# denyingmxd/CFPNet

Hardware: AMD Instinct MI355X
Metric: depth maps/sec @ 480x640 bf16 (whole job; per_gpu = value / n_gpus); abs_rel vs CPU oracle (higher is better)
Workload: dtype bf16; 1 GPU; batch=8 480x640 RGB + 8x8-zone ToF, eval forward incl. the prob output [B,256,H/2,W/2] written in the storage dtype (bf16: 2 bytes/element); layers=hist2image combine1 image x2 (CFPNet), parallelism=single GPU

## Files before the change

cfpnet_amd/csrc/conv_route.hip:

```cpp
#include "conv_route.h"

namespace {

int tile_count(int variant, int M, int Cout) {
  static const int bm[4] = {256, 256, 128, 128}, bn[4] = {16, 32, 64, 128};
  return cdiv(M, bm[variant]) * cdiv(Cout, bn[variant]);
}

int pick_splits(int variant, int M, int Cout, int K, int dtype) {
  const int bk = is16(dtype) ? 32 : 16;
  const int nk = cdiv(K, bk);
  const int tiles = tile_count(variant, M, Cout);
  if (tiles >= 128 || nk < 16) return 1;
  int s = cdiv(256, tiles);
  if (s > nk / 6) s = nk / 6;
  if (s > 32) s = 32;
  return s < 2 ? 1 : s;
}

}

static int g_force_variant = -1, g_force_splits = -1;
int g_use_v1 = 0;
int g_tput = 0;
// ... 14 lines not shown
static int chunk_x3_variant(long long M, int Cin, int Cout, bool tput) {
  if (Cin % 32 != 0) return -1;
  if (Cin == 32) {
    if (Cout <= 32) return M >= 30000 ? 45 : -1;
    if (Cout > 64 && Cout <= 128 && !tput) return (M >= 30000 && M < 200000) ? 44 : -1;
    return -1;
  }
  if (Cout > 128) return (tput && M >= 9000) ? 36 : -1;
  if (Cout > 64) return M >= 30000 ? ((!tput && M < 200000) ? 44 : 36) : -1;
  if (Cout <= 32) return M >= (tput ? 30000 : 15000) ? 45 : -1;
  if (M >= 100000) return 38;
  if (M >= 30000) return tput ? 38 : 24;
  return -1;
}
int g_chunk16 = 1;
static int chunk16_variant(long long M, int Cin, int Cout, bool tput) {
  if (Cin <= 64 || Cin % 8 != 0 || Cout <= 0 || Cout % 8 != 0 || M <= 0 || g_chunk16 == 0) return -1;
  if (g_chunk16 == 2) return Cout > 64 ? 0 : 1;
  if (M >= 30000 && M < 200000) return 1;
  if (M >= 8000 && M < 12000) return (Cout > 128) != tput ? 1 : -1;
  return -1;
}
extern "C" int cfp_conv3x3_chunk_variant(int M, int Cin, int Cout, int in_flight) { return chunk16_variant(M, Cin, Cout, in_flight > 1); }
static bool halo_wins_s2(long long M, int Cout) { return g_halo == 2 || (g_halo == 1 && g_halo_s2 && M >= 30000 && Cout <= 160); }
static bool halo_wins(long long M, int Cout, bool tput) {
  if (g_halo == 2) return true;
  if (g_halo == 1 && tput && M >= 100000 && Cout <= 64) return true;
  return g_halo == 1 && ((M >= 300000 && (Cout <= 32 || Cout == 128)) || (M >= 100000 && Cout > 128 && Cout <= 160) ||
                         (M >= 30000 && Cout > 160 && Cout <= 256));
}
void cfp_tail_x3_debug_set(int value);
void cfp_fold_debug_set(int v);
void cfp_tail16_debug_set(int value);
void cfp_pw_rows_debug_set(int value);
void cfp_attn_apply_debug_set(int value);
void cfp_dwl3_debug_set(int value);
void cfp_dwl_wgrad_debug_set(int value);
void cfp_wgrad_debug_set(int value);
void cfp_bn_debug_set(int key, int value);
void cfp_attn_debug_set(int value);
int cfp_dw_debug_set(int key, int value);
extern "C" int cfp_debug_set(int key, int value) {
  switch (key) {
    case 3: case 4: case 5: case 6: case 9: case 10: case 11: return cfp_dw_debug_set(key, value);
    case 30: cfp_dwl3_debug_set(value); return CFP_OK;
    case 32: g_x3_occ = value; return CFP_OK;
    case 33: g_x3_small_m = value; return CFP_OK;
    case 34: g_x3_small_k = value; return CFP_OK;
    case 35: cfp_tail_x3_debug_set(value); return CFP_OK;
    case 37: cfp_fold_debug_set(value); return CFP_OK;
    case 38: cfp_attn_apply_debug_set(value); return CFP_OK;
    case 39: cfp_tail16_debug_set(value); return CFP_OK;
    case 40: g_chunk16 = value; return CFP_OK;
    case 41: cfp_pw_rows_debug_set(value); return CFP_OK;
    case 17: g_tput = value; return CFP_OK;
    case 16: g_probe = (g_probe & 16) | value; return CFP_OK;
    case 29: g_x3_ad = value; return CFP_OK;
    case 28: g_probe = (g_probe & ~16) | (value ? 16 : 0); return CFP_OK;
    case 15: g_small_s2 = value; return CFP_OK;
    case 14: g_up_halo = value; return CFP_OK;
    case 19: cfp_attn_debug_set(value); return CFP_OK;
    case 20: case 21: cfp_bn_debug_set(key, value); return CFP_OK;
    case 22: cfp_wgrad_debug_set(value); return CFP_OK;
    case 23: cfp_dwl_wgrad_debug_set(value); return CFP_OK;
    case 18: g_halo_s2 = value; return CFP_OK;
    case 12: g_halo = value; return CFP_OK;
    case 24: g_halo_x3 = value; return CFP_OK;
    case 25: g_bin_head_x3_rows = value; return CFP_OK;
    case 26: g_x3_ln_fused = value; return CFP_OK;
    case 27: conv3x3_halo_debug_odd_pitch(value); return CFP_OK;
    case 13: conv3x3_halo_debug_stages(value); return CFP_OK;
    case 0: g_force_variant = value; return CFP_OK;
    case 1: g_force_splits = value; return CFP_OK;
    case 2: g_use_v1 = value; return CFP_OK;
    default: cfp_set_error("cfp_debug_set: unknown key"); return CFP_EINVAL;
  }
}

extern "C" int cfp_conv2d_variant(int M, int Cout) {
  if (Cout <= 16) return 0;
  if (Cout <= 32) return 1;
  if (Cout <= 64) return 2;
  long long t128 = (long long)cdiv(M, 128) * cdiv(Cout, 128);
  bool waste = (Cout % 128) != 0 && (Cout % 128) <= 64;
  return (t128 < 192 || waste) ? 2 : 3;
}

// ... 231 lines not shown
```

cfpnet_amd/csrc/loftr_tail.hip:

```cpp
#include "tail_core.h"

namespace {

template <typename H, int NT, int BSTAGE, int WAVES, typename AF>
__device__ __forceinline__ void tail_gemm(f32x4 (&acc)[NT], const H* __restrict__ W, int K, AF afrag, unsigned char* sB,
                                          int wave, int lane) {
  constexpr int N = NT * 16;
  constexpr int NBG = N / 8;
  constexpr int NBW = (NBG + WAVES - 1) / WAVES;
  constexpr int SST = N * 128;
  constexpr int STG = (3 * SST <= 2 * BSTAGE) ? 3 : 2;
  const int fr = lane & 15, fq = lane >> 4;
  const int rsub = lane >> 3;
  const int lc = (lane & 7) ^ rsub;
  const H* zsrc = reinterpret_cast<const H*>(g_zero16);
#pragma unroll
  for (int j = 0; j < NT; ++j) acc[j] = f32x4{0.f, 0.f, 0.f, 0.f};
  const int nk = (K + 63) >> 6;
  auto issue = [&](int ks, int st) {
    const int kk = ks * 64 + lc * 8;
    const bool kok = kk < K;
#pragma unroll
    for (int j = 0; j < NBW; ++j) {
      const int g = (j * WAVES + wave) % NBG;
// ... 129 lines not shown
    }
  }
  asm volatile("s_waitcnt lgkmcnt(0)" ::: "memory");

  constexpr int PF = D + 4;
  float* tF = reinterpret_cast<float*>(tH);
  {
    f32x4 acc[D / 16];
    tail_gemm<H, D / 16, BSTAGE, 4>(acc, p.w2, 4 * D, [&](int k) { return *reinterpret_cast<const s16x8*>(tH + fr * PH + k + fq * 8); }, sB, wave, lane);
    asm volatile("s_waitcnt lgkmcnt(0)" ::: "memory");
#pragma unroll
    for (int j = 0; j < D / 16; ++j) {
      const float bj = p.b2[j * 16 + fr];
#pragma unroll
      for (int r = 0; r < 4; ++r) tF[(fq * 4 + r) * PF + j * 16 + fr] = acc[j][r] + bj;
    }
  }
  asm volatile("s_waitcnt lgkmcnt(0)" ::: "memory");
  for (int i = lane; i < 16 * XCH; i += 64) {
    const int r = i / XCH, ch = i - r * XCH;
    const long long m = row0 + r;
    if (m < p.rows) {
      float a[8], b[8];
      Vec<float>::load(tF + r * PF + ch * 8, a);
      Vec<float>::load(tF + r * PF + ch * 8 + 4, a + 4);
      Vec<H>::load(p.xin + m * p.x_ld + ch * 8, b);
#pragma unroll
      for (int e = 0; e < 8; ++e) a[e] += b[e];
      Vec<H>::store(p.out + m * p.out_ld + ch * 8, a);
    }
  }
}

int g_tail16_waves = 0;

}

void cfp_tail16_debug_set(int value) { g_tail16_waves = value; }

static int loftr_tail_impl(const void* q, int q_ld, const float* kv, const float* ksum, const void* x, int x_ld,
                           void* out, int out_ld, const void* w_q, const void* w_merge, const void* w_mlp0, const void* w_mlp2,
                           const float* ln1_g, const float* ln1_b, const float* ln2_g, const float* ln2_b, float ln_eps,
                           int NB, int Hq, int Wq, int qth, int qtw, float v_length, float eps, int heads, int D,
                           int dtype, cfp_stream_t stream, const TailMap* map) {
  const bool x3 = dtype == CFP_F32X3;
  const int vec = x3 ? 4 : 8;
  const bool rows_ok = (long long)NB * Hq * Wq < (1ll << 31);
  CFP_REQUIRE(x3 || is16(dtype), CFP_EINVAL, "cfp_loftr_tail: bf16 / f16 or CFP_F32X3 (the plain f32 parity mode uses the unfused kernels)");
  CFP_REQUIRE((q || w_q) && kv && ksum && x && out && w_merge && w_mlp0 && w_mlp2 && ln1_g && ln1_b && ln2_g && ln2_b, CFP_EINVAL,
              "cfp_loftr_tail: null pointer (q or w_q must be given)");
  CFP_REQUIRE(NB > 0 && Hq > 0 && Wq > 0 && qth > 0 && qtw > 0 && v_length > 0.f && (rows_ok || !x3), CFP_ESHAPE, "cfp_loftr_tail: bad grid");
  CFP_REQUIRE((D == 32 || D == 64 || D == 128) && (heads == 4 || heads == 8), CFP_ESHAPE, "cfp_loftr_tail: D must be 32/64/128 and heads 4/8");
  CFP_REQUIRE((w_q || (q_ld >= D && q_ld % vec == 0)) && x_ld >= D && out_ld >= D && x_ld % vec == 0 && out_ld % vec == 0, CFP_ESHAPE,
              "cfp_loftr_tail: pitches must be >= D and multiples of " + std::to_string(vec));
  CFP_REQUIRE(aligned16(q) && aligned16(w_q) && aligned16(x) && aligned16(out) && aligned16(w_merge) && aligned16(w_mlp0) && aligned16(w_mlp2) &&
                  aligned16(kv), CFP_EINVAL, "cfp_loftr_tail: pointers must be 16-byte aligned");
  CFP_REQUIRE(rows_ok, CFP_ESHAPE, "cfp_loftr_tail: too many rows");
  hipStream_t s = reinterpret_cast<hipStream_t>(stream);
  auto params = [&](auto t, auto w) {
    return tail_params<decltype(t), decltype(w)>(q, q_ld, kv, ksum, x, x_ld, out, out_ld, w_q, w_merge, w_mlp0, w_mlp2, ln1_g, ln1_b, ln2_g, ln2_b,
                                                 ln_eps, NB, Hq, Wq, qth, qtw, v_length, eps);
  };
  auto run = [&](auto tag) {
    using H = decltype(tag);
    TailP<H, H> p = params(tag, tag);
    if (map) p.map = *map;
    return tail_pick<32, 64, 128>(D, [&](auto d) { return tail_pick<4, 8>(heads, [&](auto h) {
      return tail_pick<1, 2, 4>(tail_waves(p.rows, g_tail16_waves), [&](auto w) {
        constexpr int D_ = d, W_ = w;
        constexpr size_t lds = 2 * (2 * D_ * 128) + W_ * ((2 * (D_ + 8) + 2 * D_ + 8) * 16 * 2);
        if (map) return tail_launch<loftr_tail_kernel<H, D_, h, W_, true>, lds>(p, W_, s);
        return tail_launch<loftr_tail_kernel<H, D_, h, W_>, lds>(p, W_, s);
      }); }); });
  };
  const int rc = x3 ? loftr_tail_x3_launch(params(float{}, f16_t{}), heads, D, s) : dtype == CFP_F16 ? run(f16_t{}) : run(bf16_t{});
  CFP_REQUIRE(rc == 0, CFP_EHIP, x3 ? "cfp_loftr_tail: f16x3 launch failed" : "cfp_loftr_tail: launch failed");
  return cfp_check_launch("cfp_loftr_tail");
}

extern "C" int cfp_loftr_tail(const void* q, int q_ld, const float* kv, const float* ksum, const void* x, int x_ld,
                              void* out, int out_ld, const void* w_q, const void* w_merge, const void* w_mlp0, const void* w_mlp2,
                              const float* ln1_g, const float* ln1_b, const float* ln2_g, const float* ln2_b, float ln_eps,
                              int NB, int Hq, int Wq, int qth, int qtw, float v_length, float eps, int heads, int D,
                              int dtype, cfp_stream_t stream) {
  return loftr_tail_impl(q, q_ld, kv, ksum, x, x_ld, out, out_ld, w_q, w_merge, w_mlp0, w_mlp2, ln1_g, ln1_b, ln2_g, ln2_b, ln_eps, NB, Hq, Wq, qth, qtw,
                         v_length, eps, heads, D, dtype, stream, nullptr);
}

extern "C" int cfp_loftr_tail_x2i(const float* kv, const float* ksum, void* tok, int tok_ld, int H, int W, int sy, int sx,
                                  const void* w_q, const void* w_merge, const void* w_mlp0, const void* w_mlp2,
                                  const float* ln1_g, const float* ln1_b, const float* ln2_g, const float* ln2_b, float ln_eps,
                                  int NB, int gh, int gw, int p1, int p2, const uint8_t* zone_valid, int zn, int accumulate,
                                  float v_length, float eps, int heads, int D, int dtype, cfp_stream_t stream) {
  CFP_REQUIRE(is16(dtype), CFP_EINVAL, "cfp_loftr_tail_x2i: bf16 / f16 only");
  CFP_REQUIRE(tok && w_q, CFP_EINVAL, "cfp_loftr_tail_x2i: null pointer (the kernel projects q itself: w_q must be given)");
  CFP_REQUIRE(H > 0 && W > 0 && p1 > 0 && p2 > 0 && (long long)NB * H * W < (1ll << 31), CFP_ESHAPE, "cfp_loftr_tail_x2i: bad token map");
  CFP_REQUIRE(!zone_valid || (zn > 0 && gh <= zn * p1 && gw <= zn * p2), CFP_ESHAPE, "cfp_loftr_tail_x2i: zone grid smaller than the query grid");
  TailMap map;
  map.zone_valid = zone_valid; map.H = H; map.W = W; map.sy = sy; map.sx = sx; map.zn = zn; map.p1 = p1; map.p2 = p2; map.accumulate = accumulate;
  return loftr_tail_impl(nullptr, 0, kv, ksum, tok, tok_ld, tok, tok_ld, w_q, w_merge, w_mlp0, w_mlp2, ln1_g, ln1_b, ln2_g, ln2_b, ln_eps, NB, gh, gw,
                         p1, p2, v_length, eps, heads, D, dtype, stream, &map);
}

extern "C" int cfp_lkpm_tail(const void* t, int t_ld, const void* xin, int x_ld, void* out, int out_ld, const void* w1, const float* b1,
                             const void* w2, const float* b2, const float* ln_g, const float* ln_b, float ln_eps, int rows, int D, int dtype,
                             cfp_stream_t stream) {
  const bool x3 = dtype == CFP_F32X3;
  const int vec = x3 ? 4 : 8;
  CFP_REQUIRE(x3 || is16(dtype), CFP_EINVAL, "cfp_lkpm_tail: bf16 / f16 or CFP_F32X3 (the plain f32 parity mode uses the unfused kernels)");
  CFP_REQUIRE(t && xin && out && w1 && b1 && w2 && b2 && ln_g && ln_b, CFP_EINVAL, "cfp_lkpm_tail: null pointer");
  CFP_REQUIRE(rows > 0 && (D == 32 || D == 64 || D == 128), CFP_ESHAPE, "cfp_lkpm_tail: D must be 32/64/128");
  CFP_REQUIRE(t_ld >= D && x_ld >= D && out_ld >= D && t_ld % vec == 0 && x_ld % vec == 0 && out_ld % vec == 0, CFP_ESHAPE,
              "cfp_lkpm_tail: pitches must be >= D and multiples of " + std::to_string(vec));
  CFP_REQUIRE(aligned16(t) && aligned16(xin) && aligned16(out) && aligned16(w1) && aligned16(w2), CFP_EINVAL, "cfp_lkpm_tail: pointers must be 16-byte aligned");
  hipStream_t s = reinterpret_cast<hipStream_t>(stream);
  auto params = [&](auto tt, auto w) {
    return lkpm_params<decltype(tt), decltype(w)>(t, t_ld, xin, x_ld, out, out_ld, w1, b1, w2, b2, ln_g, ln_b, ln_eps, rows);
  };
  auto run = [&](auto tag) {
    using H = decltype(tag);
    const LkpmP<H, H> p = params(tag, tag);
    return tail_pick<32, 64, 128>(D, [&](auto d) {
      constexpr int D_ = d;
      constexpr size_t lds = 2 * (2 * D_ * 128) + 4 * (((D_ + 8) + (4 * D_ + 8)) * 16 * 2);
      return tail_launch<lkpm_tail_kernel<H, D_>, lds>(p, 4, s);
    });
  };
  const int rc = x3 ? lkpm_tail_x3_launch(params(float{}, f16_t{}), D, s) : dtype == CFP_F16 ? run(f16_t{}) : run(bf16_t{});
  CFP_REQUIRE(rc == 0, CFP_EHIP, x3 ? "cfp_lkpm_tail: f16x3 launch failed" : "cfp_lkpm_tail: launch failed");
  return cfp_check_launch("cfp_lkpm_tail");
}
```

cfpnet_amd/engine.py:

```python
from __future__ import annotations

import math
import os
from typing import Dict, List, Optional, Sequence, Tuple

import torch

from . import hip, ops, spec
from .geometry import FUSION_SCALES, FusionGeometry, gsa_keys, static_zone_key, zone_records as _zone_records
from .ops import Act

_BN_EPS = 1e-5


def _same_pad(size: int, k: int, s: int) -> Tuple[int, int]:
    total = max((math.ceil(size / s) - 1) * s + k - size, 0)
    return total // 2, total - total // 2


_STREAMS: Dict = {}
_CONCURRENT: Dict[str, list] = {}


def concurrent_streams(device, want: int = 4, pool: int = 16) -> list:
# ... 54 lines not shown
        self.base_resolution = tuple(base_resolution)
        self.fusion = spec.fusion_table(self.base_resolution)
        if not torch.cuda.is_available():
            raise RuntimeError("cfpnet_amd.Engine needs a GPU: the product path has no CPU fallback")
        assert dtype in (torch.bfloat16, torch.float16, torch.float32)
        self.layer_names = list(layer_names)
        self.n_bins, self.min_val, self.max_val = n_bins, float(min_val), float(max_val)
        self.norm = {"linear": 0, "softmax": 1, "sigmoid": 2}[norm]
        self.change_embedding, self.no_skip_inside, self.stem_act = change_embedding, no_skip_inside, stem_act
        self.dtype, self.device = dtype, torch.device(device)
        assert not x3 or dtype == torch.float32, "x3 is a matrix-math mode of float32 storage"
        self.x3 = bool(x3)
        self.cdt = hip.F32X3 if self.x3 else ops.DT[dtype]
        self.tickets = self.x3 and os.environ.get("CFP_SPLITK_TICKETS", "0") == "1"
        self.zone_sample_num = zone_sample_num
        self.weights2 = os.environ.get("CFP_WEIGHTS2", "0") == "1"
        self.diffuse_cin = os.environ.get("CFP_DIFFUSE_CIN", "1") == "1"
        self.mbconv_fused = os.environ.get("CFP_MBCONV_FUSED", "0") == "1"
        self.pw_rows = os.environ.get("CFP_PW_ROWS", "1") != "0"
        self.se2 = dtype in (torch.bfloat16, torch.float16) and os.environ.get("CFP_SE2", "1") == "1"
        self.se2_x3 = os.environ.get("CFP_SE2_X3", "1") if self.x3 else "0"
        self._dbg_round = {}
        for item in filter(None, os.environ.get("CFP_DEBUG_ROUND", "").split(",")):
            n, d = item.split(":")
            self._dbg_round[n] = {"f16": torch.float16, "bf16": torch.bfloat16}[d]
        self.up_fused = os.environ.get("CFP_UP_FUSED", "4")
        self.up_fused_x3 = os.environ.get("CFP_UP_FUSED_X3", "")
        self.cat_pad = os.environ.get("CFP_CAT_PAD", "1") == "1" and not self.up_fused_x3
        self.lkpm_fused = os.environ.get("CFP_LKPM_FUSED", "1") != "0"
        self.tail_q = os.environ.get("CFP_TAIL_Q", "1") == "1"
        self.kv_project = os.environ.get("CFP_KV_PROJECT", "1") == "1"
        self.x2i_inplace = os.environ.get("CFP_X2I_INPLACE", "1") == "1"
        self.lkpm_min_rows = int(os.environ.get("CFP_LKPM_MIN_ROWS", "30000"))
        self.sr_ln_fused = os.environ.get("CFP_SR_LN_FUSED", "1") == "1"
        self.head_fused = os.environ.get("CFP_HEAD_FUSED", "1") != "0"
        self.head_conv0 = os.environ.get("CFP_HEAD_CONV0", "1") != "0"
        self.er_fused = os.environ.get("CFP_ER_FUSED", "12")
        hl = os.environ.get("CFP_HEAD_HILO", "00")
        self.head_hilo = (hl[0] == "1", hl[1] == "1")
        self.half = dtype in (torch.bfloat16, torch.float16)
        self.ve = 8 if self.half else 4
        self.P: Dict[str, torch.Tensor] = {}
        self._plans: Dict[tuple, dict] = {}
        self._graph = None
        self._splitk_ws: Optional[torch.Tensor] = None
        self._capturing = False
        self._side = _shared_stream(self.device, "side")
        self._lane = 0
        self.use_side_stream = os.environ.get("CFP_NO_SIDE_STREAM", "0") != "1"
        self._lane_streams: Dict[int, Tuple[torch.cuda.Stream, torch.cuda.Stream]] = {}
        self._lanes_active = 1
        self._slots = None
        self._slot_next = 0
        self._lane_ws: Dict[int, torch.Tensor] = {}
        self.load_state_dict(state_dict)

    def _dev(self, t: torch.Tensor, dtype=None) -> torch.Tensor:
        return t.detach().to(device=self.device, dtype=dtype or torch.float32).contiguous()

    def _pack_conv(self, w: torch.Tensor, w2: bool = False) -> torch.Tensor:
        w = w.detach().float()
        if w.dim() == 2:
            w = w[:, :, None, None]
        elif w.dim() == 3:
            w = w[:, :, :, None]
        co, ci, kh, kw = w.shape
# ... 1023 lines not shown
```

cfpnet_amd/hip.py:

```python
from __future__ import annotations

import ctypes as C
import os
from typing import Optional

_HERE = os.path.dirname(os.path.abspath(__file__))
LIB_PATH = os.environ.get("CFP_HIP_LIB") or os.path.join(_HERE, "libcfpnet_hip.so")

F32, BF16, F16 = 0, 1, 2
F32X3 = 3
ACT_NONE, ACT_RELU, ACT_LRELU, ACT_SILU, ACT_GELU, ACT_SIGMOID = range(6)
TOF_SAMPLE_UNIFORM, TOF_SAMPLE_ICDF = 0, 1
HEAD_WOUT_HILO, HEAD_RAM_HILO = 1, 2
UNC_STD, UNC_ENTROPY, UNC_PMAX = 0, 1, 2
SPARS_STD, SPARS_ENTROPY, SPARS_PMAX, SPARS_ORACLE_RMSE, SPARS_ORACLE_ABSREL = range(5)
RENDER_DEPTH, RENDER_GT, RENDER_ABS_ERR, RENDER_REL_ERR = range(4)
REGION_ALL, REGION_FOV_IN, REGION_FOV_OUT, REGION_ZONE_VALID, REGION_ZONE_INVALID = range(5)
CONV_PER_IMAGE, CONV_W2, CONV_IN_FLIGHT, CONV_X3, CONV_WS_TICKETS = 1, 2, 4, 8, 16
CONV_TICKET_BYTES = 4096

_p, _i, _f, _sz, _ll = C.c_void_p, C.c_int, C.c_float, C.c_size_t, C.c_longlong

SIGNATURES = {
    "cfp_version": (_i, []),
# ... 117 lines not shown
    "cfp_dwconv3x3_dgrad": (_i, [_p, _i, _p, _p, _i] + [_i] * 11 + [_p]),
    "cfp_dwconv3x3_wgrad_ws_bytes": (_sz, [_i]),
    "cfp_dwconv3x3_wgrad": (_i, [_p, _i, _p, _i, _p] + [_i] * 9 + [_f, _i, _p, _sz, _p]),
    "cfp_dwconv3x3_wgrad_deferred": (_i, [_p, _i, _p, _i, _p] + [_i] * 9 + [_f, _i, _p, _sz, _p, _p]),
    "cfp_index_rows": (_i, [_p, _i, _p, _p, _i, C.c_longlong, _i, _i, _i, _p]),
    "cfp_resize_bilinear_bwd": (_i, [_p, _i, _p, _i, _i, _i, _i, _i, _i, _i, _i, _i, _p]),
    "cfp_bin_centers": (_i, [_p, _f, _f, _p, _p, _i, _i, _p]),
    "cfp_bin_centers_bwd": (_i, [_p, _f, _f, _p, _i, _i, _p]),
    "cfp_softmax_expect_ws_bytes": (_sz, [_i, _i, _i]),
    "cfp_softmax_expect": (_i, [_p, _i, _p, _p, _p, _p, _i, _p, _i, _i, _i, _i, _p, _sz, _p]),
    "cfp_linattn_state_bytes": (_sz, [_i, _i, _i]),
    "cfp_linattn_ws_bytes": (_sz, [_i, _i, _i, _i, _i]),
    "cfp_linattn_fwd": (_i, [_p, _i, _p, _i, _p, _i, _p, _i, _p, _i, _i, _i, _i, _i, _f, _i, _p, _sz, _p]),
    "cfp_linattn_bwd": (_i, [_p, _i, _p, _i, _p, _i, _p, _i, _p, _p, _i, _p, _i, _p, _i, _i, _i, _i, _i, _i, _f, _i, _p, _sz, _p]),
    "cfp_linattn_fwd_dev": (_i, [_p, _i, _p, _i, _p, _i, _p, _i, _p, _i, _i, _i, _i, _i, _f, _i, _p, _sz, _p, _p]),
    "cfp_linattn_bwd_dev": (_i, [_p, _i, _p, _i, _p, _i, _p, _i, _p, _p, _i, _p, _i, _p, _i, _i, _i, _i, _i, _i, _f, _i, _p, _sz, _p, _p]),
    "cfp_zone_crop": (_i, [_p, _i, _p, _p, _i] + [_i] * 7 + [_i, _p]),
    "cfp_zone_crop_bwd": (_i, [_p, _i, _p, _p, _i] + [_i] * 7 + [_i, _p]),
    "cfp_zone_paste": (_i, [_p, _i, _p, _i, _p, _p, _i] + [_i] * 7 + [_i, _p]),
    "cfp_zone_paste_bwd": (_i, [_p, _i, _p, _p, _i] + [_i] * 7 + [_i, _p]),
    "cfp_zone_rect_rows": (_i, [_p, _i, _p, _p, _i] + [_i] * 6 + [_i, _p]),
    "cfp_dwconv_large_wgrad_ws_bytes": (_sz, [_i, _i, _i, _i, _i]),
    "cfp_dwconv_large_wgrad": (_i, [_p, _i, _p, _i, _p, _i, _i, _i, _i, _i, _f, _i, _p, _sz, _p]),
    "cfp_row_normalize": (_i, [_p, _p, _p, _i, _i, _p]),
    "cfp_add_rowtable_dev": (_i, [_p, _i, _p, _p, _i, _i, _i, _i, _i, _i, _i, _p, _i, _p]),
    "cfp_rowtable_grad_dev": (_i, [_p, _i, _p, _i, _i, _i, _i, _i, _i, _p, _f, _i, _p]),
    "cfp_nyu_augment": (_i, [_p, _p, _i, _i, _i, _p, _p, _p, _i, _i, C.POINTER(C.c_float), C.POINTER(C.c_float), _p, _p, _p]),
    "cfp_nyu_rotate": (_i, [_p, _p, _p, _p, _i, _i, _i, _p, _p]),
    "cfp_bin_regressor": (_i, [_p, _i, _f] + [_p] * 7 + [_f, _f, _i, _p, _p, _i, _i, _i, _i, _p]),
    "cfp_bin_softmax": (_i, [_p, _i, _p, _p, _p, _i, _i, _i, _i, _p]),
    "cfp_bin_softmax_stats": (_i, [_p, _i, _p, _p, _p, _p, _i, _i, _i, _i, _p]),
    "cfp_conv3x3_mean": (_i, [_p, _i, _p, _i, _p, _p, _p, _i, _i, _i, _i, _i, _i, _p]),
    "cfp_lkpm_tail": (_i, [_p, _i, _p, _i, _p, _i, _p, _p, _p, _p, _p, _p, _f, _i, _i, _i, _p]),
    "cfp_mbconv_plan": (_i, [_i, _i, _i, _i, _i, _p, _p]),
    "cfp_mbconv_expand_dw": (_i, [_p, _i, _p, _p, _p, _p, _p, _p, _p, _i, _p, _i, _i, _i, _i, _i, _i, _p]),
    "cfp_conv3x3_pw_fused_variant": (_i, [_i] * 5),
    "cfp_conv3x3_chunk_variant": (_i, [_i] * 4),
    "cfp_conv3x3_pw_fused": (_i, [_p, _i, _p, _p, _p, _i, _p, _p, _p, _i, _p, _i, _p, _i] + [_i] * 12 + [_p]),
    "cfp_pw_rows_fits": (_i, [_ll, _i, _i, _i, _i, _i]),
    "cfp_pw_rows_groups": (_i, [_ll, _i, _i, _p]),
    "cfp_pw_rows": (_i, [_p, _i, _p, _p, _p, _i, _p, _i, _ll, _i, _i, _i, _i, _p]),
    "cfp_hist_encoder": (_i, [_p, _p, _p, _p, _p, _p, _p, _p, _p, _i, _i, _i, _p]),
    "cfp_depth_head_fused": (_i, [_p, _i, _p, _p, _p, _p, _p, _p, _p, _p, _p, _i, _i, _i, _i, _i, _p]),
    "cfp_bin_head_fused": (_i, [_p, _i, _p, _p, _p, _p, _p, _i, _i, _i, _i, _p]),
    "cfp_depth_head_conv0_fused": (_i, [_p, _i, _p, _p, _p, _p, _p, _p, _p, _p, _p, _p, _p, _i, _i, _i, _i, _i, _p]),
    "cfp_depth_head_fused_stats": (_i, [_p, _i, _p, _p, _p, _p, _p, _p, _p, _p, _p, _p, _i, _i, _i, _i, _i, _p]),
    "cfp_bin_head_fused_stats": (_i, [_p, _i, _p, _p, _p, _p, _p, _p, _i, _i, _i, _i, _p]),
}

class WgradJob(C.Structure):
    _fields_ = [("slabs", C.c_void_p), ("dw", C.c_void_p), ("db", C.c_void_p), ("n", C.c_longlong), ("n_dw", C.c_longlong),
                ("nsplit", C.c_int), ("ew", C.c_int), ("beta", C.c_float), ("beta_b", C.c_float)]


_lib: Optional[C.CDLL] = None


def load() -> C.CDLL:
    global _lib
    if _lib is not None:
        return _lib
    if not os.path.exists(LIB_PATH):
        raise RuntimeError(
            f"{LIB_PATH} not found: build the HIP extension first "
            f"(`python -c 'import __graft_entry__ as g; g.build()'` or `make -C cfpnet_amd/csrc`). "
            "There is no CPU fallback for the product path.")
# ... 28 lines not shown
```

include/cfpnet_hip.h:

```cpp
#ifndef CFPNET_HIP_H
#define CFPNET_HIP_H

#include <stddef.h>
#include <stdint.h>

#ifdef __cplusplus
extern "C" {
#endif

typedef void* cfp_stream_t;

enum { CFP_OK = 0, CFP_EINVAL = -1, CFP_ESHAPE = -2, CFP_EHIP = -3 };
enum { CFP_F32 = 0, CFP_BF16 = 1, CFP_F16 = 2 };
enum { CFP_F32X3 = 3 };
enum { CFP_TOF_SAMPLE_UNIFORM = 0, CFP_TOF_SAMPLE_ICDF = 1 };
enum { CFP_ACT_NONE = 0, CFP_ACT_RELU = 1, CFP_ACT_LRELU = 2, CFP_ACT_SILU = 3, CFP_ACT_GELU = 4, CFP_ACT_SIGMOID = 5 };

int cfp_version(void);
const char* cfp_last_error(void);

int cfp_conv2d_nhwc(const void* in, int in_ld, const void* w, const float* scale, const float* shift,
                    const void* residual, int res_ld, void* out, int out_ld,
                    int B, int H, int W, int Cin, int Cout, int KH, int KW, int stride,
                    int pad_t, int pad_l, int Ho, int Wo, int act, int dtype,
// ... 125 lines not shown
                       int NB, int gh, int gw, int p1, int p2, const uint8_t* zone_valid, int zn, int accumulate,
                       float v_length, float eps, int heads, int D, int dtype, cfp_stream_t stream);

int cfp_resize_bilinear(const void* src, int src_ld, int Hs, int Ws, int sy0, int sx0, int sh, int sw,
                        void* dst, int dst_ld, int Hd, int Wd, int dy0, int dx0, int dh, int dw,
                        const uint8_t* zone_valid, int zn, int p1, int p2, int accumulate,
                        int B, int C, int dtype, cfp_stream_t stream);

int cfp_resize_bilinear_dev(const void* src, int src_ld, int Hs, int Ws, void* dst, int dst_ld, int Hd, int Wd,
                            const int* rec, int rec_side, const uint8_t* zone_valid, int zn, int p1, int p2,
                            int accumulate, int B, int C, int dtype, cfp_stream_t stream);

int cfp_add_rowtable(const void* in, int in_ld, const float* table, void* out, int out_ld, int rows, int C,
                     int H, int W, int Wt, int oy, int ox, int dtype, cfp_stream_t stream);

int cfp_upsample_cat_conv3x3(const void* low, int low_ld, int Hs, int Ws, int Cup, const void* skip, int skip_ld, int Cskip,
                             const void* w, const float* scale, const float* shift, void* out, int out_ld, int B, int H, int W,
                             int Cout, int act, int dtype, cfp_stream_t stream);

int cfp_copy_rows(const void* in, int in_ld, void* out, int out_ld, int rows, int C, int dtype, cfp_stream_t stream);
int cfp_copy_rows2(const void* in0, int in0_ld, void* out0, int out0_ld, int C0, const void* in1, int in1_ld, void* out1, int out1_ld,
                   int C1, int rows, int dtype, cfp_stream_t stream);

int cfp_rgb_to_nhwc8(const float* rgb, void* out, int B, int H, int W, int dtype, cfp_stream_t stream);
int cfp_rgb_to_nhwc8_hilo(const float* rgb, void* out, int B, int H, int W, int dtype, cfp_stream_t stream);
int cfp_scalar_to_rows8(const float* in, void* out, int rows, int dtype, cfp_stream_t stream);

int cfp_hist_encoder(const float* hist, const float* blob, const int* layout, void* out0, void* out1, void* out2,
                     const float* pe0, const float* pe1, const float* pe2, int n_pe, int R, int dtype, cfp_stream_t stream);

int cfp_lkpm_tail(const void* t, int t_ld, const void* xin, int x_ld, void* out, int out_ld, const void* w1, const float* b1,
                  const void* w2, const float* b2, const float* ln_g, const float* ln_b, float ln_eps, int rows, int D, int dtype,
                  cfp_stream_t stream);

int cfp_bin_regressor(const float* partial, int nsplit, float inv_hw, const float* w1x1_t,
                      const float* w0_t, const float* b0, const float* w1_t, const float* b1,
                      const float* w2_t, const float* b2, float min_val, float max_val, int norm,
                      float* edges, float* centers, int B, int C, int hidden, int nbins, cfp_stream_t stream);

int cfp_conv3x3_mean(const float* partial, int nsplit, const void* in, int in_ld, const float* w, const float* bias, float* msum,
                     int B, int H, int W, int C, int Cout, int dtype, cfp_stream_t stream);

int cfp_bin_softmax(const void* logits, int ld, const float* centers, void* prob, float* pred,
                    int B, int HW, int nbins, int dtype, cfp_stream_t stream);

enum { CFP_UNC_STD = 0, CFP_UNC_ENTROPY = 1, CFP_UNC_PMAX = 2 };
int cfp_bin_softmax_stats(const void* logits, int ld, const float* centers, void* prob, float* pred, float* stats,
                          int B, int HW, int nbins, int dtype, cfp_stream_t stream);

enum { CFP_HEAD_WOUT_HILO = 1, CFP_HEAD_RAM_HILO = 2 };
int cfp_depth_head_fused(const void* x, int x_ld, const void* w3, const float* scale3, const float* shift3,
                         const void* wout_perm, const float* bias_out, const float* centers, void* prob, float* pred,
                         void* ram_out, int B, int H, int W, int flags, int dtype, cfp_stream_t stream);
int cfp_depth_head_fused_stats(const void* x, int x_ld, const void* w3, const float* scale3, const float* shift3,
                               const void* wout_perm, const float* bias_out, const float* centers, void* prob, float* pred,
                               float* stats, void* ram_out, int B, int H, int W, int flags, int dtype, cfp_stream_t stream);

int cfp_depth_head_conv0_fused(const void* t, int t_ld, const void* w0, const float* scale0, const float* shift0, const void* w3,
                               const float* scale3, const float* shift3, const void* wout_perm, const float* bias_out,
                               const float* centers, void* prob, float* pred, int B, int H, int W, int flags, int dtype,
                               cfp_stream_t stream);

int cfp_bin_head_fused(const void* x, int x_ld, const void* w, const float* bias, const float* centers,
                       void* prob, float* pred, int B, int HW, int Cin, int dtype, cfp_stream_t stream);
int cfp_bin_head_fused_stats(const void* x, int x_ld, const void* w, const float* bias, const float* centers,
                             void* prob, float* pred, float* stats, int B, int HW, int Cin, int dtype, cfp_stream_t stream);
// ... 284 lines not shown
```

Measured before the change: 4133 maps/s.

## Add front-loaded weight-resident LoFTR and LKPM tail kernels for D=32 16-bit

Adds new fused tail kernels for the LoFTR and LKPM transformer tails. At block start they DMA every layer's weights into LDS in one go, then run the whole GEMM chain per 16-row wave tile with no per-k-step ring pipeline. The kv/ksum attention state and the residual input are held in registers, which aims to remove repeated weight streaming and ring synchronisation overhead. The path applies only to D=32, 16-bit dtypes and large row counts, and uses a fixed four waves. It adds a large specialised code path and more register pressure.

```diff
diff --git a/cfpnet_amd/csrc/conv_route.hip b/cfpnet_amd/csrc/conv_route.hip
--- a/cfpnet_amd/csrc/conv_route.hip
+++ b/cfpnet_amd/csrc/conv_route.hip
@@ -70,6 +70,7 @@
 void cfp_tail_x3_debug_set(int value);
 void cfp_fold_debug_set(int v);
 void cfp_tail16_debug_set(int value);
+void cfp_tail_front_debug_set(int value);
 void cfp_pw_rows_debug_set(int value);
 void cfp_attn_apply_debug_set(int value);
 void cfp_dwl3_debug_set(int value);
@@ -91,6 +92,7 @@
     case 39: cfp_tail16_debug_set(value); return CFP_OK;
     case 40: g_chunk16 = value; return CFP_OK;
     case 41: cfp_pw_rows_debug_set(value); return CFP_OK;
+    case 42: cfp_tail_front_debug_set(value); return CFP_OK;
     case 17: g_tput = value; return CFP_OK;
     case 16: g_probe = (g_probe & 16) | value; return CFP_OK;
     case 29: g_x3_ad = value; return CFP_OK;
diff --git a/cfpnet_amd/csrc/loftr_tail.hip b/cfpnet_amd/csrc/loftr_tail.hip
--- a/cfpnet_amd/csrc/loftr_tail.hip
+++ b/cfpnet_amd/csrc/loftr_tail.hip
@@ -185,11 +185,357 @@
   }
 }
 
+constexpr int FRONT_WAVES = 4;
+
+__device__ __forceinline__ int front_pack_pos(int c, int row) { return c ^ ((0x78 >> (2 * ((row >> 2) & 3))) & 3); }
+
+template <typename H, int N, int K, bool PACK>
+__device__ __forceinline__ void front_issue(const H* __restrict__ W, unsigned char* dst, int wave, int lane) {
+  static_assert(!PACK || K == 32, "packed slabs hold 32 k");
+  constexpr int RPG = PACK ? 16 : 8;
+  constexpr int NBG = N / RPG, TOT = NBG * ((K + 63) / 64);
+  constexpr int WAVES = FRONT_WAVES;
+  static_assert(TOT % WAVES == 0, "every wave issues the same number of loads");
+  const int rsub = PACK ? lane >> 2 : lane >> 3;
+  const int lc = PACK ? front_pack_pos(lane & 3, rsub) : (lane & 7) ^ rsub;
+  const H* zsrc = reinterpret_cast<const H*>(g_zero16);
+#pragma unroll
+  for (int j = 0; j < TOT / WAVES; ++j) {
+    const int idx = j * WAVES + wave, ks = idx / NBG, g = idx % NBG;
+    const int kk = ks * 64 + lc * 8;
+    glds16(kk < K ? W + (long long)(g * RPG + rsub) * K + kk : zsrc, dst + ks * (N * 128) + g * 1024);
+  }
+}
+constexpr int front_slab_bytes(int N, int K, bool pack) { return pack ? N * 64 : N * 128 * ((K + 63) / 64); }
+
+template <typename H, int NT, int K, bool PACK, typename AF>
+__device__ __forceinline__ void front_gemm(f32x4 (&acc)[NT], const unsigned char* sW, AF afrag, int lane) {
+  constexpr int SST = NT * 16 * 128;
+  const int fr = lane & 15, fq = lane >> 4;
+#pragma unroll
+  for (int j = 0; j < NT; ++j) acc[j] = f32x4{0.f, 0.f, 0.f, 0.f};
+#pragma unroll
+  for (int k = 0; k < K; k += 32) {
+    const s16x8 a = afrag(k);
+    const int ks = k >> 6, sub = (k >> 5) & 1;
+#pragma unroll
+    for (int j = 0; j < NT; ++j) {
+      const unsigned char* bp = PACK ? sW + (j * 16 + fr) * 64 + front_pack_pos(fq, fr) * 16
+                                     : sW + ks * SST + (j * 16 + fr) * 128 + (((sub * 4 + fq) ^ (fr & 7)) * 16);
+      acc[j] = mfma16<H>(a, *reinterpret_cast<const s16x8*>(bp), acc[j]);
+    }
+  }
+}
+
+__device__ __forceinline__ void front_landed() {
+  asm volatile("s_waitcnt vmcnt(0) lgkmcnt(0)" ::: "memory");
+  __builtin_amdgcn_s_barrier();
+  asm volatile("" ::: "memory");
+}
+
+template <int NT>
+__device__ __forceinline__ void front_ln_coeffs(float (&g)[NT], float (&bt)[NT], const float* __restrict__ gamma, const float* __restrict__ beta, int fr) {
+#pragma unroll
+  for (int j = 0; j < NT; ++j) { g[j] = gamma[j * 16 + fr]; bt[j] = beta[j * 16 + fr]; }
+}
+template <int NT, typename ROUND_T>
+__device__ __forceinline__ void front_layernorm(f32x4 (&acc)[NT], const float (&g)[NT], const float (&bt)[NT], float eps) {
+  constexpr float inv_n = 1.f / (float)(NT * 16);
+#pragma unroll
+  for (int r = 0; r < 4; ++r) {
+    float s = 0.f;
+#pragma unroll
+    for (int j = 0; j < NT; ++j) {
+      acc[j][r] = to_f32<ROUND_T>(from_f32<ROUND_T>(acc[j][r]));
+      s += acc[j][r];
+    }
+    s = row16_sum(s);
+    const float mean = s * inv_n;
+    float qq = 0.f;
+#pragma unroll
+    for (int j = 0; j < NT; ++j) { const float dlt = acc[j][r] - mean; qq = fmaf(dlt, dlt, qq); }
+    qq = row16_sum(qq);
+    const float rstd = rsqrtf(qq * inv_n + eps);
+#pragma unroll
+    for (int j = 0; j < NT; ++j) acc[j][r] = (acc[j][r] - mean) * rstd * g[j] + bt[j];
+  }
+}
+template <typename T>
+__device__ __forceinline__ long long front_attn_group(const TailP<T, T>& p, long long mm) {
+  const unsigned t = fd_div((unsigned)mm, p.fwq), xq = (unsigned)mm - t * (unsigned)p.Wq;
+  const unsigned b = fd_div(t, p.fhq), yq = t - b * (unsigned)p.Hq;
+  return ((long long)b * p.ggy + fd_div(yq, p.fqth)) * p.ggx + fd_div(xq, p.fqtw);
+}
+template <typename T, int d>
+__device__ __forceinline__ void front_attn_head(const TailP<T, T>& p, const float (&qv)[d], const float* kv, const float* ks, bool ok, T* msg) {
+  float o[d];
+#pragma unroll
+  for (int j = 0; j < d; ++j) o[j] = 0.f;
+  float z = 0.f;
+#pragma unroll
+  for (int i = 0; i < d; ++i) {
+    const float qe = elu1(qv[i]);
+    z = fmaf(qe, ks[i], z);
+#pragma unroll
+    for (int j = 0; j < d; j += 4) {
+      const f32x4 kk = *reinterpret_cast<const f32x4*>(kv + i * d + j);
+      o[j] = fmaf(qe, kk[0], o[j]); o[j + 1] = fmaf(qe, kk[1], o[j + 1]);
+      o[j + 2] = fmaf(qe, kk[2], o[j + 2]); o[j + 3] = fmaf(qe, kk[3], o[j + 3]);
+    }
+  }
+  const float zi = 1.f / (z + p.eps);
+#pragma unroll
+  for (int j = 0; j < d; ++j) {
+    const T v = from_f32<T>(o[j] * zi * p.v_length);
+    msg[j] = ok ? v : T(0);
+  }
+}
+template <typename T, int D, int PA>
+__device__ __forceinline__ void front_row_layernorm(T* tile, const float (&gq)[D / 4], const float (&bq)[D / 4], float eps, int fr, int fq) {
+  constexpr int Q = D / 4, E = Vec<T>::N;
+  T* row = tile + fr * PA + fq * Q;
+  float v[Q];
+#pragma unroll
+  for (int c = 0; c < Q; c += E) Vec<T>::load(row + c, v + c);
+  float s = 0.f;
+#pragma unroll
+  for (int c = 0; c < Q; ++c) s += v[c];
+  s += __shfl_xor(s, 16, 64); s += __shfl_xor(s, 32, 64);
+  const float mean = s * (1.f / (float)D);
+  float qq = 0.f;
+#pragma unroll
+  for (int c = 0; c < Q; ++c) { const float dl = v[c] - mean; qq = fmaf(dl, dl, qq); }
+  qq += __shfl_xor(qq, 16, 64); qq += __shfl_xor(qq, 32, 64);
+  const float rstd = rsqrtf(qq * (1.f / (float)D) + eps);
+#pragma unroll
+  for (int c = 0; c < Q; c += E) {
+    float o[E];
+#pragma unroll
+    for (int e = 0; e < E; ++e) o[e] = (v[c + e] - mean) * rstd * gq[c + e] + bq[c + e];
+    Vec<T>::store(row + c, o);
+  }
+}
+
+template <int D> struct FrontLoftr {
+  static constexpr int OFF_Q = 0, OFF_M = OFF_Q + front_slab_bytes(D, D, false), OFF_0 = OFF_M + front_slab_bytes(D, D, false),
+                       OFF_2 = OFF_0 + front_slab_bytes(2 * D, 2 * D, false), W_LDS = OFF_2 + front_slab_bytes(D, 2 * D, false);
+  static constexpr int WAVE_LDS = (2 * (D + 8) + 2 * D + 8) * 16 * 2;
+  static constexpr size_t LDS = (size_t)W_LDS + FRONT_WAVES * WAVE_LDS;
+  static_assert(W_LDS <= 65536, "LDS-DMA destinations stay below 64 KB");
+  static_assert(D != 32 || (W_LDS == 20480 && 4 * LDS <= 163840), "D = 32: 20 KB of weights, four workgroups per CU as the streaming kernel");
+};
+
+template <typename H, int D, int HEADS, bool MAP>
+__global__ __launch_bounds__(64 * FRONT_WAVES) void loftr_tail_front_kernel(TailP<H, H> p) {
+  using L = FrontLoftr<D>;
+  constexpr int WAVES = FRONT_WAVES;
+  constexpr int PA = D + 8, PH = 2 * D + 8, NT = D / 16, d = D / HEADS;
+  static_assert(d <= 8, "kv / ksum of the lane's (row, head slots) are held in registers");
+  extern __shared__ __attribute__((aligned(16))) unsigned char smem[];
+  const int tid = threadIdx.x;
+  const int lane = tid & 63;
+  const int wave = __builtin_amdgcn_readfirstlane(tid >> 6);
+  const int fr = lane & 15, fq = lane >> 4;
+  H* tMsg = reinterpret_cast<H*>(smem + L::W_LDS + wave * L::WAVE_LDS);
+  H* tX = tMsg + 16 * PA;
+  H* tH = tX + 16 * PA;
+  const long long row0 = (long long)blockIdx.x * (16 * WAVES) + wave * 16;
+  const bool own_q = p.wq != nullptr;
+
+  if (own_q) front_issue<H, D, D, false>(p.wq, smem + L::OFF_Q, wave, lane);
+  front_issue<H, D, D, false>(p.wm, smem + L::OFF_M, wave, lane);
+  front_issue<H, 2 * D, 2 * D, false>(p.w0, smem + L::OFF_0, wave, lane);
+  front_issue<H, D, 2 * D, false>(p.w2, smem + L::OFF_2, wave, lane);
+  float g1[NT], b1[NT], g2[NT], b2[NT];
+  front_ln_coeffs<NT>(g1, b1, p.g1, p.b1, fr);
+  front_ln_coeffs<NT>(g2, b2, p.g2, p.b2, fr);
+  const long long m = row0 + fr;
+  const bool ok = m < p.rows;
+  const long long mm = ok ? m : 0;
+  const long long grp = front_attn_group(p, mm);
+  __attribute__((aligned(16))) float kvr[HEADS / 4][d * d], ksr[HEADS / 4][d];
+#pragma unroll
+  for (int hs = 0; hs < HEADS / 4; ++hs) {
+    const float* __restrict__ kv = p.kv + (grp * HEADS + fq + 4 * hs) * d * d;
+    const float* __restrict__ ks = p.ksum + (grp * HEADS + fq + 4 * hs) * d;
+#pragma unroll
+    for (int i = 0; i < d * d; i += 4) *reinterpret_cast<f32x4*>(&kvr[hs][i]) = *reinterpret_cast<const f32x4*>(kv + i);
+#pragma unroll
+    for (int i = 0; i < d; ++i) ksr[hs][i] = ks[i];
+  }
+  if constexpr (MAP) tail_tile_load_mapped<H, D, PA>(tX, p, row0, lane);
+  else tail_tile_load<H, D, PA>(tX, p.x, p.x_ld, row0, p.rows, lane);
+  front_landed();
+
+  if (own_q) {
+    f32x4 acc[NT];
+    front_gemm<H, NT, D, false>(acc, smem + L::OFF_Q, [&](int k) { return *reinterpret_cast<const s16x8*>(tX + fr * PA + k + fq * 8); }, lane);
+#pragma unroll
+    for (int j = 0; j < NT; ++j)
+#pragma unroll
+      for (int r = 0; r < 4; ++r) tH[(fq * 4 + r) * PH + j * 16 + fr] = from_f32<H>(acc[j][r]);
+    asm volatile("s_waitcnt lgkmcnt(0)" ::: "memory");
+  }
+
+#pragma unroll
+  for (int hs = 0; hs < HEADS / 4; ++hs) {
+    const int h = fq + 4 * hs;
+    float qv[d];
+    if (own_q) tail_load_f32<H, d, true>(tH + fr * PH + h * d, qv);
+    else tail_load_f32<H, d, false>(p.q + mm * p.q_ld + h * d, qv);
+    front_attn_head<H, d>(p, qv, kvr[hs], ksr[hs], ok, tMsg + fr * PA + h * d);
+  }
+  asm volatile("s_waitcnt lgkmcnt(0)" ::: "memory");
+  __builtin_amdgcn_sched_barrier(0);
+
+  {
+    f32x4 acc[NT];
+    front_gemm<H, NT, D, false>(acc, smem + L::OFF_M, [&](int k) { return *reinterpret_cast<const s16x8*>(tMsg + fr * PA + k + fq * 8); }, lane);
+    front_layernorm<NT, H>(acc, g1, b1, p.ln_eps);
+#pragma unroll
+    for (int j = 0; j < NT; ++j)
+#pragma unroll
+      for (int r = 0; r < 4; ++r) tMsg[(fq * 4 + r) * PA + j * 16 + fr] = from_f32<H>(acc[j][r]);
+  }
+  asm volatile("s_waitcnt lgkmcnt(0)" ::: "memory");
+  __builtin_amdgcn_sched_barrier(0);
+
+  {
+    f32x4 acc[2 * NT];
+    front_gemm<H, 2 * NT, 2 * D, false>(acc, smem + L::OFF_0, [&](int k) {
+      const H* src = k < D ? tX + fr * PA + k : tMsg + fr * PA + (k - D);
+      return *reinterpret_cast<const s16x8*>(src + fq * 8);
+    }, lane);
+#pragma unroll
+    for (int j = 0; j < 2 * NT; ++j)
+#pragma unroll
+      for (int r = 0; r < 4; ++r) tH[(fq * 4 + r) * PH + j * 16 + fr] = from_f32<H>(fmaxf(acc[j][r], 0.f));
+  }
+  asm volatile("s_waitcnt lgkmcnt(0)" ::: "memory");
+  __builtin_amdgcn_sched_barrier(0);
+
+  {
+    f32x4 acc[NT];
+    front_gemm<H, NT, 2 * D, false>(acc, smem + L::OFF_2, [&](int k) { return *reinterpret_cast<const s16x8*>(tH + fr * PH + k + fq * 8); }, lane);
+    front_layernorm<NT, H>(acc, g2, b2, p.ln_eps);
+#pragma unroll
+    for (int j = 0; j < NT; ++j)
+#pragma unroll
+      for (int r = 0; r < 4; ++r) {
+        const int row = fq * 4 + r, col = j * 16 + fr;
+        tMsg[row * PA + col] = from_f32<H>(acc[j][r] + to_f32<H>(tX[row * PA + col]));
+      }
+  }
+  asm volatile("s_waitcnt lgkmcnt(0)" ::: "memory");
+  if constexpr (MAP) tail_tile_store_mapped<H, D, PA>(p, tMsg, row0, lane);
+  else tail_tile_store<H, D, PA>(p.out, p.out_ld, tMsg, row0, p.rows, lane);
+}
+
+template <int D> struct FrontLkpm {
+  static constexpr bool PACK = D == 32;
+  static constexpr int OFF_1 = 0, OFF_2 = front_slab_bytes(4 * D, D, PACK), W_LDS = OFF_2 + front_slab_bytes(D, 4 * D, false);
+  static constexpr int WAVE_LDS = ((D + 8) + (4 * D + 8)) * 16 * 2;
+  static constexpr size_t LDS = (size_t)W_LDS + FRONT_WAVES * WAVE_LDS;
+  static_assert(W_LDS <= 65536, "LDS-DMA destinations stay below 64 KB");
+  static_assert(D != 32 || LDS <= 2 * (2 * D * 128) + 4 * WAVE_LDS, "D = 32: no more LDS than the streaming kernel (four workgroups per CU)");
+};
+
+template <typename H, int D>
+__global__ __launch_bounds__(64 * FRONT_WAVES) void lkpm_tail_front_kernel(LkpmP<H, H> p) {
+  using L = FrontLkpm<D>;
+  constexpr int WAVES = FRONT_WAVES;
+  constexpr int PA = D + 8, PH = 4 * D + 8, Q = D / 4;
+  constexpr int XCH = D / 8, NX = 16 * XCH / 64;
+  extern __shared__ __attribute__((aligned(16))) unsigned char smem[];
+  const int tid = threadIdx.x;
+  const int lane = tid & 63;
+  const int wave = __builtin_amdgcn_readfirstlane(tid >> 6);
+  const int fr = lane & 15, fq = lane >> 4;
+  H* tA = reinterpret_cast<H*>(smem + L::W_LDS + wave * L::WAVE_LDS);
+  H* tH = tA + 16 * PA;
+  const long long row0 = (long long)blockIdx.x * (16 * WAVES) + wave * 16;
+
+  front_issue<H, 4 * D, D, L::PACK>(p.w1, smem + L::OFF_1, wave, lane);
+  front_issue<H, D, 4 * D, false>(p.w2, smem + L::OFF_2, wave, lane);
+  float lg[Q], lb[Q], c1[4 * D / 16], c2[D / 16];
+#pragma unroll
+  for (int c = 0; c < Q; ++c) { lg[c] = p.lg[fq * Q + c]; lb[c] = p.lb[fq * Q + c]; }
+#pragma unroll
+  for (int j = 0; j < 4 * D / 16; ++j) c1[j] = p.b1[j * 16 + fr];
+#pragma unroll
+  for (int j = 0; j < D / 16; ++j) c2[j] = p.b2[j * 16 + fr];
+  u32x4 xr[NX];
+#pragma unroll
+  for (int c = 0; c < NX; ++c) {
+    const int i = lane + c * 64, r = i / XCH, ch = i - r * XCH;
+    xr[c] = u32x4{0u, 0u, 0u, 0u};
+    if (row0 + r < p.rows) xr[c] = *reinterpret_cast<const u32x4*>(p.xin + (row0 + r) * p.x_ld + ch * 8);
+  }
+  tail_tile_load<H, D, PA>(tA, p.t, p.t_ld, row0, p.rows, lane);
+  front_landed();
+  front_row_layernorm<H, D, PA>(tA, lg, lb, p.ln_eps, fr, fq);
+  asm volatile("s_waitcnt lgkmcnt(0)" ::: "memory");
+
+#pragma unroll
+  for (int half = 0; half < 2; ++half) {
+    f32x4 acc[2 * D / 16];
+    front_gemm<H, 2 * D / 16, D, L::PACK>(acc, smem + L::OFF_1 + half * front_slab_bytes(2 * D, D, L::PACK),
+                                          [&](int k) { return *reinterpret_cast<const s16x8*>(tA + fr * PA + k + fq * 8); }, lane);
+#pragma unroll
+    for (int j = 0; j < 2 * D / 16; ++j) {
+      const float bj = c1[half * (2 * D / 16) + j];
+#pragma unroll
+      for (int r = 0; r < 4; ++r)
+        tH[(fq * 4 + r) * PH + half * 2 * D + j * 16 + fr] = from_f32<H>(act_c16<CFP_ACT_GELU>(acc[j][r] + bj));
+    }
+  }
+  asm volatile("s_waitcnt lgkmcnt(0)" ::: "memory");
+
+  constexpr int PF = D + 4;
+  float* tF = reinterpret_cast<float*>(tH);
+  {
+    f32x4 acc[D / 16];
+    front_gemm<H, D / 16, 4 * D, false>(acc, smem + L::OFF_2, [&](int k) { return *reinterpret_cast<const s16x8*>(tH + fr * PH + k + fq * 8); }, lane);
+    asm volatile("s_waitcnt lgkmcnt(0)" ::: "memory");
+#pragma unroll
+    for (int j = 0; j < D / 16; ++j)
+#pragma unroll
+      for (int r = 0; r < 4; ++r) tF[(fq * 4 + r) * PF + j * 16 + fr] = acc[j][r] + c2[j];
+  }
+  asm volatile("s_waitcnt lgkmcnt(0)" ::: "memory");
+#pragma unroll
+  for (int c = 0; c < NX; ++c) {
+    const int i = lane + c * 64, r = i / XCH, ch = i - r * XCH;
+    const long long m = row0 + r;
+    if (m < p.rows) {
+      float a[8], b[8];
+      Vec<float>::load(tF + r * PF + ch * 8, a);
+      Vec<float>::load(tF + r * PF + ch * 8 + 4, a + 4);
+      Vec<H>::load(reinterpret_cast<const H*>(&xr[c]), b);
+#pragma unroll
+      for (int e = 0; e < 8; ++e) a[e] += b[e];
+      Vec<H>::store(p.out + m * p.out_ld + ch * 8, a);
+    }
+  }
+}
+
 int g_tail16_waves = 0;
+int g_tail_front = 1;
+
+int tail_front_waves(int kernel, long long rows, int D, int heads, int dtype) {
+  if (g_tail_front == 0 || !is16(dtype) || D != 32 || kernel < 0 || kernel > 2) return 0;
+  if (kernel != 2 && (g_tail16_waves == 1 || g_tail16_waves == 2 || g_tail16_waves == 4)) return 0;
+  if (kernel != 2 && heads != 4 && heads != 8) return 0;
+  if (g_tail_front != 2 && rows < 8192) return 0;
+  return FRONT_WAVES;
+}
 
 }
 
 void cfp_tail16_debug_set(int value) { g_tail16_waves = value; }
+void cfp_tail_front_debug_set(int value) { g_tail_front = value; }
+
+extern "C" int cfp_tail_frontload(int kernel, long long rows, int D, int heads, int dtype) { return tail_front_waves(kernel, rows, D, heads, dtype); }
 
 static int loftr_tail_impl(const void* q, int q_ld, const float* kv, const float* ksum, const void* x, int x_ld,
                            void* out, int out_ld, const void* w_q, const void* w_merge, const void* w_mlp0, const void* w_mlp2,
@@ -218,6 +564,12 @@
     using H = decltype(tag);
     TailP<H, H> p = params(tag, tag);
     if (map) p.map = *map;
+    if (tail_front_waves(map ? 1 : 0, p.rows, D, heads, dtype))
+      return tail_pick<32>(D, [&](auto d) { return tail_pick<4, 8>(heads, [&](auto h) {
+        constexpr int D_ = d;
+        if (map) return tail_launch<loftr_tail_front_kernel<H, D_, h, true>, FrontLoftr<D_>::LDS>(p, FRONT_WAVES, s);
+        return tail_launch<loftr_tail_front_kernel<H, D_, h, false>, FrontLoftr<D_>::LDS>(p, FRONT_WAVES, s);
+      }); });
     return tail_pick<32, 64, 128>(D, [&](auto d) { return tail_pick<4, 8>(heads, [&](auto h) {
       return tail_pick<1, 2, 4>(tail_waves(p.rows, g_tail16_waves), [&](auto w) {
         constexpr int D_ = d, W_ = w;
@@ -273,6 +625,11 @@
   auto run = [&](auto tag) {
     using H = decltype(tag);
     const LkpmP<H, H> p = params(tag, tag);
+    if (tail_front_waves(2, rows, D, 0, dtype))
+      return tail_pick<32>(D, [&](auto d) {
+        constexpr int D_ = d;
+        return tail_launch<lkpm_tail_front_kernel<H, D_>, FrontLkpm<D_>::LDS>(p, FRONT_WAVES, s);
+      });
     return tail_pick<32, 64, 128>(D, [&](auto d) {
       constexpr int D_ = d;
       constexpr size_t lds = 2 * (2 * D_ * 128) + 4 * (((D_ + 8) + (4 * D_ + 8)) * 16 * 2);
diff --git a/cfpnet_amd/engine.py b/cfpnet_amd/engine.py
--- a/cfpnet_amd/engine.py
+++ b/cfpnet_amd/engine.py
@@ -110,6 +110,8 @@
         self.kv_project = os.environ.get("CFP_KV_PROJECT", "1") == "1"
         self.x2i_inplace = os.environ.get("CFP_X2I_INPLACE", "1") == "1"
         self.lkpm_min_rows = int(os.environ.get("CFP_LKPM_MIN_ROWS", "30000"))
+        if os.environ.get("CFP_TAIL_FRONT", "1") == "0":
+            hip.load().cfp_debug_set(42, 0)
         self.sr_ln_fused = os.environ.get("CFP_SR_LN_FUSED", "1") == "1"
         self.head_fused = os.environ.get("CFP_HEAD_FUSED", "1") != "0"
         self.head_conv0 = os.environ.get("CFP_HEAD_CONV0", "1") != "0"
diff --git a/cfpnet_amd/hip.py b/cfpnet_amd/hip.py
--- a/cfpnet_amd/hip.py
+++ b/cfpnet_amd/hip.py
@@ -173,6 +173,7 @@
     "cfp_bin_softmax_stats": (_i, [_p, _i, _p, _p, _p, _p, _i, _i, _i, _i, _p]),
     "cfp_conv3x3_mean": (_i, [_p, _i, _p, _i, _p, _p, _p, _i, _i, _i, _i, _i, _i, _p]),
     "cfp_lkpm_tail": (_i, [_p, _i, _p, _i, _p, _i, _p, _p, _p, _p, _p, _p, _f, _i, _i, _i, _p]),
+    "cfp_tail_frontload": (_i, [_i, _ll, _i, _i, _i]),
     "cfp_mbconv_plan": (_i, [_i, _i, _i, _i, _i, _p, _p]),
     "cfp_mbconv_expand_dw": (_i, [_p, _i, _p, _p, _p, _p, _p, _p, _p, _i, _p, _i, _i, _i, _i, _i, _i, _p]),
     "cfp_conv3x3_pw_fused_variant": (_i, [_i] * 5),
diff --git a/include/cfpnet_hip.h b/include/cfpnet_hip.h
--- a/include/cfpnet_hip.h
+++ b/include/cfpnet_hip.h
@@ -181,6 +181,8 @@
 int cfp_lkpm_tail(const void* t, int t_ld, const void* xin, int x_ld, void* out, int out_ld, const void* w1, const float* b1,
                   const void* w2, const float* b2, const float* ln_g, const float* ln_b, float ln_eps, int rows, int D, int dtype,
                   cfp_stream_t stream);
+
+int cfp_tail_frontload(int kernel, long long rows, int D, int heads, int dtype);
 
 int cfp_bin_regressor(const float* partial, int nsplit, float inv_hw, const float* w1x1_t,
                       const float* w0_t, const float* b0, const float* w1_t, const float* b1,
```

Result: no change. 4170 maps/s (median of 6 runs) (+0.9%).
